# lwowlwowl/advanced_scrapper

Hardware: AMD Instinct MI355X
Metric: article GB/s keyword-matched (S&P500 set) at 1 & 8 GPUs; % of HBM peak (higher is better)
Workload: dtype u8

## Files before the change

### advanced_scrapper_amd/csrc/kwmatch_split.hpp

```cpp
#pragma once
#include "kwmatch_fast_kernel.hpp"

namespace kw {

#ifndef FS_WAVES_CFG
#define FS_WAVES_CFG 16
#endif
#ifndef FS_MINW
#define FS_MINW 1
#endif
#ifndef FS_EQ_TRIGGER
#define FS_EQ_TRIGGER 32
#endif
#ifndef FS_AHEAD
#define FS_AHEAD 3
#endif

constexpr int FS_WAVES = FS_WAVES_CFG;
constexpr int FS_BLOCK = FS_WAVES * WAVE;
constexpr int PK_WAVES = 4;
constexpr int PK_BLOCK = PK_WAVES * WAVE;
#ifndef PK_POOL_CFG
#define PK_POOL_CFG 768
#endif
constexpr int PK_POOL = PK_POOL_CFG;
#ifndef FK_TX
#define FK_TX 1
#endif
#ifndef EK_MINW
#define EK_MINW 4
#endif
#ifndef PK_MINW
#define PK_MINW 5
#endif
constexpr int EK_WAVES = 8;
constexpr int EK_BIGQ = 64;
constexpr int EK_BLOCK = EK_WAVES * WAVE;

constexpr int FG_DOCS = 32;
#ifndef EF_TX_FLAT
#define EF_TX_FLAT 1
#endif

struct __attribute__((aligned(16))) FilterLds {
    uint32_t s1[FK_S1_WORDS];
    uint32_t p2[FK_P2_WORDS];
    uint32_t l2[FK_L2_WORDS];
    uint32_t t3[FK_T3_WORDS];
    uint32_t b2[FK_B2_WORDS];
    uint32_t dstart[FS_WAVES][FG_DOCS + 1];
    uint32_t dtitle[FS_WAVES][FG_DOCS];
    uint2 sent[FS_WAVES][2 * WAVE];
    uint32_t spos[FS_WAVES][WAVE];
};

__device__ __forceinline__ uint32_t fg_doc(const uint32_t *dstart, uint32_t nd, uint32_t r)
{
    uint32_t lo = 0, n = nd;
    while (n > 1) {
        const uint32_t h = n >> 1;
        if (dstart[lo + h] <= r) lo += h;
        n -= h;
    }
    return lo;
}

__device__ __forceinline__ uint32_t fk_b2_mul(uint32_t key)
{
    uint32_t r;
    asm("v_mul_u32_u24 %0, %1, %2" : "=v"(r) : "s"(40503u), "v"(key));
    return r;
}

__device__ __forceinline__ constexpr uint32_t fk_tbit(int j) { return (uint32_t)((j >> 2) + 8 * (j & 3)); }
__device__ __forceinline__ uint32_t fk_tpos(uint32_t b) { return ((b & 7u) << 2) + (b >> 3); }
__device__ __forceinline__ uint32_t fk_untranspose(uint32_t t)
{
    uint32_t x = (t & 0xFu) | ((t >> 4) & 0xF0u) | ((t >> 8) & 0xF00u) | ((t >> 12) & 0xF000u);
    uint32_t d = (x ^ (x >> 3)) & 0x0A0Au;
    x ^= d ^ (d << 3);
    d = (x ^ (x >> 6)) & 0x00CCu;
    x ^= d ^ (d << 6);
    return x;
}
__device__ __forceinline__ uint32_t fk_transpose16(uint32_t v)
{
    uint32_t t = 0;
#pragma unroll
    for (int j = 0; j < 16; ++j) t |= ((v >> j) & 1u) << fk_tbit(j);
    return t;
}

__device__ __forceinline__ uint32_t fk_in_box(uint32_t x, uint32_t A, uint32_t B, uint32_t N)
{
    const uint32_t t = x & 0x7F7F7F7Fu;
    return (((t + A) & ~(t + B) & ~x) | (x & N)) & 0x80808080u;
}

template <int SH>
__device__ __forceinline__ void fk_stage1(const FastTables &FT, const FilterLds &L, const uint32_t (&W)[5],
                                          uint32_t &hit, uint32_t &gate)
{
    uint32_t k[17];
#pragma unroll
    for (int j = 0; j < 16; ++j) k[j] = (j & 3) ? __builtin_amdgcn_alignbyte(W[(j >> 2) + 1], W[j >> 2], j & 3) : W[j >> 2];
    k[16] = W[4];
// ... 25 lines not shown
        for (int q = 0; q < 4; ++q) {
            const uint32_t f0 = (t[q] + FT.gate[0]) & ~(t[q] + FT.gate[1]);
            const uint32_t pr = f0 & __builtin_amdgcn_alignbyte(f1[q + 1], f1[q], 1) & 0x80808080u;
            g |= pr >> (7 - q);
        }
    } else if (SH == 2) {
        uint32_t f[5];
#pragma unroll
        for (int q = 0; q < 5; ++q) f[q] = fk_in_box(W[q], FT.gate[0], FT.gate[1], FT.gate[2]);
#pragma unroll
        for (int q = 0; q < 4; ++q) {
            const uint32_t pr = f[q] & __builtin_amdgcn_alignbyte(f[q + 1], f[q], 1);
            g |= pr >> (7 - q);
        }
    }
    uint32_t h = 0;
#pragma unroll
    for (int j = 0; j < 16; ++j) {
        const uint32_t b = __builtin_amdgcn_ubfe(sw[j], hh[j], 1);
        h |= b << fk_tbit(j);
    }
    hit = h;
    gate = g;
}

template <int SH>
__device__ __forceinline__ void fk_filter_groups(const FastTables &FT, FilterLds &L, const uint8_t *__restrict__ arena,
                                                 const int64_t *__restrict__ off, int64_t n_docs, const FastScratch &S,
                                                 int64_t region, int64_t g_lo, int64_t g_hi, int wib, uint32_t &ncand,
                                                 uint32_t &ncand2, uint32_t &ccur)
{
    const int lane = lane_id();
    const uint32_t *l2 = L.l2, *t3 = L.t3, *b2 = L.b2;
    uint32_t *dstart = L.dstart[wib], *dtitle = L.dtitle[wib];
    uint32_t *spos = L.spos[wib];
    uint32_t *cand = S.cand + (size_t)region * S.cand_cap;
    const uint32_t ccap = S.cand_cap;
    const uint32_t t3on = FT.has_t3 ? 1u : 0u;
    for (int64_t g = g_lo; g < g_hi; ++g) {
        const int64_t d0 = g * FG_DOCS;
        const int nd = (int)(n_docs - d0 < FG_DOCS ? n_docs - d0 : FG_DOCS);
        const int64_t o0 = lane <= nd ? off[2 * (d0 + lane)] : 0;
        const int64_t o1 = lane < nd ? off[2 * (d0 + lane) + 1] : 0;
        const int64_t gb = rdlane64(o0, 0), ge = rdlane64(o0, nd);
        if (ge - gb > 0x7FFFFFFFll) {
            if (lane < nd) atomicOr(&S.dflags[d0 + lane], DH_DEFER);
            continue;
        }
        if (ge <= gb) continue;
        wave_sync();
        if (lane <= nd) dstart[lane] = (uint32_t)(o0 - gb);
        if (lane < nd) dtitle[lane] = (uint32_t)(o1 - gb);
        wave_sync();
        const uint8_t *gbase = arena + (gb & ~(int64_t)15);
        const uint32_t g0 = (uint32_t)(gb & 15), gl = (uint32_t)(ge - (gb & ~(int64_t)15));
        uint32_t blk = 0;
        uint32_t kdoc = 0;
        bool ghdr = true;
        const uint32_t glast = (gl - 1u) & ~15u;
        auto load = [&](uint4 &v, uint32_t &w, uint32_t tb) {
            const uint32_t a = tb + 16u * (uint32_t)lane, e = tb + 1024u;
            v = *(const uint4 *)(gbase + (a < glast ? a : glast));
            w = *(const uint32_t *)(gbase + (e < glast ? e : glast));
        };
        auto round_at = [&](uint32_t n, uint32_t r, uint32_t key) {
            const bool act = (uint32_t)lane < n;
            const uint32_t b4 = (uint32_t)lds_bit(l2, fk_l2_index(key));
            const uint32_t pr = (uint32_t)lds_bit(L.p2, fk_b2_index(key));
            const uint32_t b3 = pr & t3on & (uint32_t)lds_bit(t3, fk_t3_index(key));
            const uint32_t bb = pr & (uint32_t)lds_bit(b2, fk_b2h_index(key));
            const uint32_t fl = b4 | (b3 << 1) | (bb << 2);
            {
                const uint32_t r0 = (uint32_t)__builtin_amdgcn_readfirstlane((int)r);
                while (dstart[kdoc + 1] <= r0) ++kdoc;
            }
            bool keep = act && fl != 0u;
            uint32_t k = kdoc, pd = 0;
            if (keep) {
                while (dstart[k + 1] <= r) ++k;
                pd = r - dstart[k];
                keep = pd < (1u << 24);
            }
            const uint64_t pm = __ballot(keep);
            if (pm) {
                if (ghdr) {
                    if (lane == 0 && ccur < ccap) cand[ccur] = (uint32_t)g << 3;
                    ++ccur;
                    ghdr = false;
                }
                const uint32_t kk = ccur + mbcnt(pm);
                if (keep && kk < ccap) cand[kk] = (pd << 8) | (k << 3) | fl;
            }
            const uint32_t np = (uint32_t)__popcll(pm);
            ccur += np;
            ncand2 += (lane == 0) ? np : 0u;
        };
        uint2 *sent = L.sent[wib];
        uint32_t eh = 0, en = 0;
        uint32_t qn = 0, qr = 0, qx0 = 0, qx1 = 0;
        auto round = [&]() {
            wave_sync();
            const bool ein = (uint32_t)lane < en;
            const uint2 ent = ein ? sent[(eh + (uint32_t)lane) & (2u * WAVE - 1u)] : make_uint2(0u, 0u);
            const int c = __popc(ent.y);
            int tot;
            const int ex = wave_excl_scan_dpp(c, &tot);
            const uint64_t tm = __ballot(ein && ex + c <= WAVE);
            const int E = __popcll(tm);
            if ((tm >> lane) & 1ull) {
                uint32_t m = fk_untranspose(ent.y);
                uint32_t o = (uint32_t)ex;
                while (m) {
                    spos[o++] = ent.x + (uint32_t)(__ffs(m) - 1);
                    m &= m - 1u;
                }
            }
            const uint32_t n = (uint32_t)__shfl(ex + c, E - 1, WAVE);
            eh = (eh + (uint32_t)E) & (2u * WAVE - 1u);
            en -= (uint32_t)E;
            wave_sync();
            const uint32_t r = spos[lane];
            wave_sync();
            uint32_t x0 = 0, x1 = 0;
#if defined(FS_TIMING_SKIP) && FS_TIMING_SKIP == 2
            x0 = r * 0x9E3779B1u;
#else
            if ((uint32_t)lane < n) {
                const int64_t a0 = (gb + (int64_t)r) & ~(int64_t)3;
                x0 = *(const uint32_t *)(arena + a0);
                x1 = *(const uint32_t *)(arena + a0 + 4);
            }
#endif
            if (qn) round_at(qn, qr, __builtin_amdgcn_alignbyte(qx1, qx0, (uint32_t)(gb + qr) & 3u));
            qn = n;
            qr = r;
            qx0 = x0;
            qx1 = x1;
        };
        auto tile = [&](const uint4 &v, uint32_t w4, uint32_t tb) {
            const uint32_t lp = tb + 16u * (uint32_t)lane;
            uint32_t W[5];
            W[0] = v.x;
            W[1] = v.y;
            W[2] = v.z;
            W[3] = v.w;
            {
                const uint32_t nx = (uint32_t)__shfl_down((int)v.x, 1, WAVE);
                W[4] = lane == WAVE - 1 ? w4 : nx;
            }
            uint32_t valid = 0xFFFFu;
            if (tb < g0 || tb + 1024u > gl) {
                const int32_t rlo = (int32_t)(g0 - lp), rhi = (int32_t)(gl - lp);
                const int jlo = rlo <= 0 ? 0 : (rlo >= 16 ? 16 : rlo);
                const int jhi = rhi <= 0 ? 0 : (rhi >= 16 ? 16 : rhi);
                valid = (jhi > jlo) ? (((1u << jhi) - 1u) & ~((1u << jlo) - 1u)) : 0u;
            }
            const uint32_t rel = lp - g0;
            if ((W[0] | W[1] | W[2] | W[3]) & 0x80808080u) {
                uint32_t hb = 0;
#pragma unroll
                for (int k = 0; k < 4; ++k) {
                    const uint32_t x = (W[k] >> 7) & 0x01010101u;
                    hb |= ((x & 1u) | ((x >> 7) & 2u) | ((x >> 14) & 4u) | ((x >> 21) & 8u)) << (4 * k);
                }
                hb &= valid;
                while (hb) {
                    const uint32_t r = rel + (uint32_t)(__ffs(hb) - 1);
                    const uint32_t k = fg_doc(dstart, (uint32_t)nd, r);
                    const uint32_t tb2 = dtitle[k];
                    const bool title = r >= tb2;
                    atomicOr(&S.dflags[d0 + k], title ? DH_NA1 : DH_NA0);
                    const uint32_t fend = title ? dstart[k + 1] : tb2;
                    const int64_t skip = (int64_t)fend - (int64_t)(int32_t)rel;
                    hb &= skip >= 16 ? 0u : ~((1u << (uint32_t)skip) - 1u);
                }
            }
            uint32_t hit, gate;
            fk_stage1<SH>(FT, L, W, hit, gate);
            const uint32_t tvalid = valid == 0xFFFFu ? 0x0F0F0F0Fu : fk_transpose16(valid);
            const uint32_t sm = (hit | gate) & tvalid;
            ncand += (uint32_t)__popc(sm);
            const uint64_t em = __ballot(sm != 0u);
            if (!em) return;
            if (sm != 0u) sent[(eh + en + mbcnt(em)) & (2u * WAVE - 1u)] = make_uint2(rel, sm);
            en += (uint32_t)__popcll(em);
#if defined(FS_TIMING_SKIP) && FS_TIMING_SKIP == 1
            en = 0;
#endif
            while (en >= (uint32_t)FS_EQ_TRIGGER) round();
        };
        uint4 v[FS_AHEAD];
        uint32_t w[FS_AHEAD];
#pragma unroll
        for (int k = 0; k < FS_AHEAD; ++k) {
            load(v[k], w[k], blk + 1024 * k);
            __builtin_amdgcn_sched_barrier(0);
        }
        for (bool more = true; more;) {
#pragma unroll
            for (int k = 0; k < FS_AHEAD; ++k) {
                if (blk >= gl) { more = false; break; }
                tile(v[k], w[k], blk);
                load(v[k], w[k], blk + 1024 * FS_AHEAD);
                blk += 1024;
            }
        }
        while (en) round();
        if (qn) round_at(qn, qr, __builtin_amdgcn_alignbyte(qx1, qx0, (uint32_t)(gb + qr) & 3u));
    }
}

__global__ __launch_bounds__(FS_BLOCK, FS_MINW) void kw_filter_kernel(FastTables FT, const uint8_t *__restrict__ arena,
                                                             const int64_t *__restrict__ off, int64_t n_docs,
                                                             FastScratch S)
{
    __shared__ FilterLds L;
    {
        const uint4 *src = (const uint4 *)FT.s1;
        uint4 *dst = (uint4 *)L.s1;
        for (int i = threadIdx.x; i < FK_S1_WORDS / 4; i += FS_BLOCK) dst[i] = src[i];
    }
    for (int i = threadIdx.x; i < FK_P2_WORDS; i += FS_BLOCK) L.p2[i] = FT.p2[i];
    for (int i = threadIdx.x; i < FK_L2_WORDS; i += FS_BLOCK) L.l2[i] = FT.l2[i];
    for (int i = threadIdx.x; i < FK_T3_WORDS; i += FS_BLOCK) L.t3[i] = FT.t3[i];
    for (int i = threadIdx.x; i < FK_B2_WORDS; i += FS_BLOCK) L.b2[i] = FT.b2[i];
    __syncthreads();
    const int lane = lane_id();
    const int wib = threadIdx.x / WAVE;
    const int64_t wave = (int64_t)blockIdx.x * FS_WAVES + wib;
    const int64_t n_waves = (int64_t)gridDim.x * FS_WAVES;
    uint32_t ncand = 0, ncand2 = 0;
    const int64_t n_groups = (n_docs + FG_DOCS - 1) / FG_DOCS;
    const int64_t K = S.chunk_groups;
    const int64_t n_chunks = (n_groups + K - 1) / K;
    const bool gate_one = FT.gate[0] == FT.gate[3] && FT.gate[1] == FT.gate[4] && FT.gate[2] == FT.gate[5];
    for (int64_t c = S.dyn ? fk_next_group(S.gnext, true, 0, 0) : wave; c < n_chunks;
         c = fk_next_group(S.gnext, S.dyn, c, n_waves)) {
        uint32_t ccur = 0;
        const int64_t g_lo = c * K, g_hi = g_lo + K < n_groups ? g_lo + K : n_groups;
        if (!FT.has_short)
            fk_filter_groups<0>(FT, L, arena, off, n_docs, S, c, g_lo, g_hi, wib, ncand, ncand2, ccur);
        else if (gate_one)
            fk_filter_groups<2>(FT, L, arena, off, n_docs, S, c, g_lo, g_hi, wib, ncand, ncand2, ccur);
        else if (FT.gate[2] == 0u && FT.gate[5] == 0u)
            fk_filter_groups<3>(FT, L, arena, off, n_docs, S, c, g_lo, g_hi, wib, ncand, ncand2, ccur);
        else
            fk_filter_groups<1>(FT, L, arena, off, n_docs, S, c, g_lo, g_hi, wib, ncand, ncand2, ccur);
        if (lane == 0) {
            S.ccnt[c] = ccur;
            if (ccur > S.cand_cap) {
                atomicOr(&S.status[0], ST_CAND_OVERFLOW);
                atomicMax(&S.cmax[0], ccur);
            }
        }
    }
    unsigned long long c1 = ncand;
#pragma unroll
    for (int dd = 32; dd >= 1; dd >>= 1) c1 += __shfl_xor(c1, dd, WAVE);
    if (lane == 0) {
        atomicAdd(&S.stats[0], c1);
        atomicAdd(&S.stats[8], (unsigned long long)ncand2);
// ... 198 lines not shown
                } while (0);
                const uint64_t pm = __ballot(pass);
                if (pass) {
                    const uint32_t k = pn + (uint32_t)__builtin_popcountll(pm & ((1ull << lane) - 1));
                    if (k < (uint32_t)PK_POOL) { pool[k] = item; pown[k] = (uint8_t)owner; }
                    atomicAdd(&scnt[owner], 1u);
                }
                pn += (uint32_t)__builtin_popcountll(pm);
            }
            wave_sync();
        }
        const uint32_t nmine = scnt[lane];
        int itotal;
        const int iex = wave_excl_scan_dpp((int)nmine, &itotal);
        const bool ovf = pn > (uint32_t)PK_POOL || icur + (uint32_t)itotal > icap;
        const uint64_t withm = __ballot(nmine > 0);
        if (withm) {
            const uint64_t below = (1ull << lane) - 1;
            const uint64_t prevm = withm & below;
            const uint32_t pdoc = (uint32_t)__shfl((int)doc, prevm ? 63 - __builtin_clzll(prevm) : 0, WAVE);
            const uint32_t prev_doc = prevm ? pdoc : last_doc;
            if (nmine > 0) {
                if (doc != prev_doc) S.hdr[doc].x = ibase + icur + (uint32_t)iex;
                atomicAdd(f ? &S.ncnt[doc].y : &S.ncnt[doc].x, nmine);
                if (ovf) atomicOr(&S.dflags[doc], DH_DEFER);
            }
            last_doc = (uint32_t)__shfl((int)doc, 63 - __builtin_clzll(withm), WAVE);
            if (!ovf) {
                scnt[lane] = icur + (uint32_t)iex;
                wave_sync();
                for (uint32_t j = (uint32_t)lane; j < pn; j += WAVE) {
                    const uint32_t idx = atomicAdd(&scnt[pown[j]], 1u);
                    if (idx < icap) items[idx] = pool[j];
                }
                wave_sync();
            }
        }
        icur += (uint32_t)itotal;
        scnt[lane] = 0;
        wave_sync();
    }
    if (lane == 0 && icur > icap && S.item_grow) {
        atomicOr(&S.status[0], ST_CAND_OVERFLOW);
        atomicMax(&S.cmax[1], icur);
    }
    wave_sync();
    }
    unsigned long long a = nanchor;
#pragma unroll
    for (int dd = 32; dd >= 1; dd >>= 1) a += __shfl_xor(a, dd, WAVE);
    if (lane == 0) atomicAdd(&S.stats[1], a);
}

__device__ __forceinline__ uint32_t fk_edge_flags(const FastTables &FT, const FastDoc &D)
{
    const int lane = lane_id();
    const int f = lane >> 1;
    const int64_t fb = f ? D.t1 : D.t0, fe = f ? D.t2 : D.t1;
    bool e = false;
    if (lane < 4 && fe - fb >= (int64_t)EDGE_MIN_M + 1) {
        const int64_t a = (lane & 1) ? fe - 8 : fb;
        const uint64_t k = (uint64_t)ld_u32_unaligned(D.arena, a) | ((uint64_t)ld_u32_unaligned(D.arena, a + 4) << 32);
        const uint32_t idx = fk_edge_index(k);
        e = (((lane & 1) ? FT.edge_suf : FT.edge_pre)[idx >> 5] >> (idx & 31u)) & 1u;
    }
    const uint64_t em = __ballot(e);
    return ((em & 3ull) ? DH_EDGE0 : 0u) | ((em & 12ull) ? DH_EDGE1 : 0u);
}

__device__ __forceinline__ uint32_t fk_edge_flags_key(const FastTables &FT, const FastDoc &D, uint64_t k)
{
    const int lane = lane_id();
    const int f = lane >> 1;
    const int64_t fb = f ? D.t1 : D.t0, fe = f ? D.t2 : D.t1;
    bool e = false;
    if (lane < 4 && fe - fb >= (int64_t)EDGE_MIN_M + 1) {
        const uint32_t idx = fk_edge_index(k);
        e = (((lane & 1) ? FT.edge_suf : FT.edge_pre)[idx >> 5] >> (idx & 31u)) & 1u;
    }
    const uint64_t em = __ballot(e);
    return ((em & 3ull) ? DH_EDGE0 : 0u) | ((em & 12ull) ? DH_EDGE1 : 0u);
}

#ifndef TX_MINW
#define TX_MINW 8
#endif
constexpr int TX_WAVES = 4;
constexpr int TX_BLOCK = TX_WAVES * WAVE;
constexpr uint32_t TX_NONE = 0xFFFFFFFFu;
constexpr unsigned long long TX_SLAB = 16384;

__device__ __forceinline__ uint64_t tx_bytes(int64_t l0, int64_t l1)
{
    return ((uint64_t)(l0 + l1) + 16ull + 15ull) & ~15ull;
}
__device__ __forceinline__ uint32_t tx_nchunks(int64_t fb, int64_t fe) { return (uint32_t)((fe - (fb & ~(int64_t)15) + 15) >> 4) + 1u; }

__device__ __forceinline__ uint32_t tx_marker(const uint32_t *txk, const uint32_t *txv, uint32_t cp)
{
    uint32_t s = (cp * 0x9E3779B1u) >> 24;
    for (int k = 0; k < 256; ++k) {
        const uint32_t kk = txk[s];
        if (kk == cp) return txv[s];
        if (kk == 0xFFFFFFFFu) break;
        s = (s + 1) & 255u;
    }
    return 0x80u;
}

__device__ uint32_t tx_field(const uint32_t *txk, const uint32_t *txv, const uint8_t *__restrict__ a, int64_t fb, int64_t fe,
                             uint8_t *__restrict__ out, uint32_t o0, uint16_t *__restrict__ chunk, uint8_t *stg)
{
    const int lane = lane_id();
    const int64_t base = fb & ~(int64_t)15;
    uint32_t count = 0;
    auto ld = [&](int64_t b, uint4 &v, uint32_t &w4) {
        const int64_t p = b + 16 * (int64_t)lane;
        v = p < fe ? *(const uint4 *)(a + p) : make_uint4(0u, 0u, 0u, 0u);
        w4 = (lane == WAVE - 1 && b + 1024 < fe) ? *(const uint32_t *)(a + b + 1024) : 0u;
    };
    uint4 vn;
    uint32_t wn;
    ld(base, vn, wn);
    for (int64_t blk = base; blk < fe; blk += 1024) {
        const int64_t lp = blk + 16 * (int64_t)lane;
        const uint4 v = vn;
        const uint32_t w4 = wn;
        if (blk + 1024 < fe) ld(blk + 1024, vn, wn);
        uint32_t W[5];
        W[0] = v.x; W[1] = v.y; W[2] = v.z; W[3] = v.w;
        W[4] = (uint32_t)__shfl_down((int)W[0], 1, WAVE);
        if (lane == WAVE - 1) W[4] = w4;
        const int64_t r0 = fb - lp, r2 = fe - lp;
        const int jlo = r0 <= 0 ? 0 : (r0 >= 16 ? 16 : (int)r0);
        const int jhi = r2 <= 0 ? 0 : (r2 >= 16 ? 16 : (int)r2);
        const uint32_t valid = (jhi > jlo) ? (((1u << jhi) - 1u) & ~((1u << jlo) - 1u)) : 0u;
        const bool asc = ((W[0] | W[1] | W[2] | W[3]) & 0x80808080u) == 0u;
        uint32_t lead = 0xFFFFu, high = 0;
        if (!asc) {
            lead = 0;
#pragma unroll
            for (int j = 0; j < 16; ++j) {
                const uint32_t b = (W[j >> 2] >> (8 * (j & 3))) & 0xFFu;
                lead |= (uint32_t)((b & 0xC0u) != 0x80u) << j;
                high |= (uint32_t)(b >= 0x80u) << j;
            }
        }
        lead &= valid;
        high &= valid;
        int total;
        const int ex = wave_excl_scan_dpp(__popc(lead), &total);
        if (chunk && lp < fe) chunk[(lp - base) >> 4] = (uint16_t)(count + (uint32_t)ex);
        wave_sync();
        const uint32_t g0 = o0 + count, g1 = g0 + (uint32_t)total, sh = g0 & 15u;
        const uint32_t k = (uint32_t)ex + sh;
        const uint32_t hl = lead & high;
        if (asc && valid == 0xFFFFu) {
            *(uint4 *)(stg + k) = v;
        } else {
#pragma unroll
            for (int j = 0; j < 16; ++j)
                if (((lead & ~hl) >> j) & 1u) stg[k + (uint32_t)__popc(lead & ((1u << j) - 1u))] = (uint8_t)(W[j >> 2] >> (8 * (j & 3)));
        }
        for (uint32_t lm = hl; lm; lm &= lm - 1) {
            const int j = __ffs(lm) - 1;
            const uint32_t b0 = (W[j >> 2] >> (8 * (j & 3))) & 0xFFu;
            const uint32_t n = (b0 >= 0xF0u) ? 4u : (b0 >= 0xE0u) ? 3u : 2u;
            uint32_t c = b0 & (0x7Fu >> n);
            for (uint32_t q = 1; q < n; ++q) {
                const int jj = j + (int)q;
                const uint32_t bk = (lp + jj < fe) ? ((W[jj >> 2] >> (8 * (jj & 3))) & 0xFFu) : 0x80u;
                c = (c << 6) | (bk & 0x3Fu);
            }
            stg[k + (uint32_t)__popc(lead & ((1u << j) - 1u))] = (uint8_t)tx_marker(txk, txv, c);
        }
        wave_sync();
        const uint32_t gb = g0 & ~15u;
        const uint32_t a0 = (g0 + 15u) & ~15u, a1 = g1 & ~15u;
        if (a0 < a1) {
            if ((uint32_t)lane < a0 - g0) out[g0 + lane] = stg[g0 - gb + lane];
            if ((uint32_t)lane < g1 - a1) out[a1 + lane] = stg[a1 - gb + lane];
            for (uint32_t q = a0 + 16u * (uint32_t)lane; q < a1; q += 16u * WAVE)
                *(uint4 *)(out + q) = *(const uint4 *)(stg + (q - gb));
        } else {
            for (uint32_t q = g0 + (uint32_t)lane; q < g1; q += WAVE) out[q] = stg[q - gb];
// ... 153 lines not shown
    for (uint32_t i = (uint32_t)lane; i < n0 + n1; i += WAVE) {
        uint64_t it = src[i];
        const bool t = i < n0;
        unsafe |= (FT.pat_info[it_pat(it)] & PI_TXUNSAFE) != 0;
        if (flags & (t ? DH_NA0 : DH_NA1))
            it = it_with_pos(it, tx_pos(D0.arena, t ? D0.t0 : D0.t1, t ? ch0 : ch1, it_pos(it)));
        items[t ? i : CAP0 + (i - n0)] = it;
    }
    if (__ballot(unsafe)) return false;
    wave_sync();
    FastDoc D;
    D.arena = S.tarena;
    D.t0 = tb;
    D.t1 = D.t0 + c0;
    D.t2 = D.t1 + c1;
    D.doc = D0.doc;
    D.l1 = (int32_t)c0;
    D.l2 = (int32_t)(c0 + c1);
    *done = fk_scan_epilogue<CAP0>(FT, S, GS, D, items, n0, n1, flags, wave, O, TC);
    return true;
}

constexpr uint32_t EK_TXBIG = 0x80000000u;

#ifndef EK_BIG_NOINLINE
#define EK_BIG_NOINLINE 0
#endif
#if EK_BIG_NOINLINE
__device__ __attribute__((noinline))
#else
__device__ __forceinline__
#endif
uint32_t epi_big_doc(const FastTables &FT, const FastScratch &S, const DevScratch &GS,
                                                          const uint8_t *__restrict__ arena, const int64_t *__restrict__ off,
                                                          uint32_t e, uint64_t *items, int64_t wave, OutCtx &O,
                                                          TaskCounts &TC)
{
    const int lane = lane_id();
    const bool tx = (e & EK_TXBIG) != 0;
    const uint32_t d = e & ~EK_TXBIG;
    const int64_t ov = lane < 3 ? off[2 * (int64_t)d + lane] : 0;
    const uint2 hv = lane == 3 ? S.hdr[d] : (lane == 4 ? S.ncnt[d] : (lane == 5 ? make_uint2(0u, S.dflags[d]) :
                                                                    make_uint2(0u, 0u)));
    FastDoc D;
    D.arena = arena;
    D.t0 = rdlane64(ov, 0);
    D.t1 = rdlane64(ov, 1);
    D.t2 = rdlane64(ov, 2);
    D.doc = d;
    D.l1 = (int32_t)(D.t1 - D.t0);
    D.l2 = (int32_t)(D.t2 - D.t0);
    const uint32_t ibeg = (uint32_t)__builtin_amdgcn_readlane((int)hv.x, 3);
    const uint32_t dfl = (uint32_t)__builtin_amdgcn_readlane((int)hv.y, 5);
    uint32_t flags = dfl & ~DH_DEFER;
    const uint32_t n0 = (uint32_t)__builtin_amdgcn_readlane((int)hv.x, 4);
    const uint32_t n1 = (uint32_t)__builtin_amdgcn_readlane((int)hv.y, 4);
    flags |= fk_edge_flags(FT, D);
    const uint64_t *src = S.items + ibeg;
    bool view = true;
    if (tx) {
        const uint4 V = S.vrec[d];
        const uint32_t c0 = V.z, c1 = V.w;
        const int64_t tb = (int64_t)(((uint64_t)(V.y & 0x7FFFFFFFu) << 32) | V.x);
        view = V.y != TX_NONE && !(dfl & DH_DEFER) &&
               !(FT.tx_unsafe_edge && (((flags & DH_NA0) && (flags & DH_EDGE0) && fk_txu_edge(FT, S.tarena + tb, c0)) ||
                                       ((flags & DH_NA1) && (flags & DH_EDGE1) && fk_txu_edge(FT, S.tarena + tb + c0, c1)))) &&
               !(FT.tx_unsafe_short && (((flags & DH_NA0) && fk_txu_short(FT, S.tarena + tb, c0)) ||
                                        ((flags & DH_NA1) && fk_txu_short(FT, S.tarena + tb + c0, c1))));
        if (view) {
            const uint64_t nb = tx_bytes(D.t1 - D.t0, D.t2 - D.t1);
            const uint16_t *ch0 = (const uint16_t *)(S.tarena + tb + nb);
            const uint16_t *ch1 = ch0 + ((flags & DH_NA0) ? tx_nchunks(D.t0, D.t1) : 0u);
            bool unsafe = false;
            for (uint32_t i = (uint32_t)lane; i < n0 + n1; i += WAVE) {
                uint64_t it = src[i];
                const bool t = i < n0;
                unsafe |= (FT.pat_info[it_pat(it)] & PI_TXUNSAFE) != 0;
                if (flags & (t ? DH_NA0 : DH_NA1))
                    it = it_with_pos(it, tx_pos(arena, t ? D.t0 : D.t1, t ? ch0 : ch1, it_pos(it)));
                items[t ? i : FK_BIG0 + (i - n0)] = it;
            }
            view = __ballot(unsafe) == 0ull;
            D.arena = S.tarena;
            D.t0 = tb;
            D.t1 = D.t0 + c0;
            D.t2 = D.t1 + c1;
            D.l1 = (int32_t)c0;
            D.l2 = (int32_t)(c0 + c1);
        }
        if (!view) {
            if (lane == 0) {
                S.dflags[d] = dfl | DH_RESOLVE;
                const uint32_t i = atomicAdd(S.res_cnt, 1u);
                if (i < S.defer_cap) S.res_list[i] = d;
            }
            wave_sync();
            return 4u;
        }
    } else {
        for (uint32_t k = (uint32_t)lane; k < n0; k += WAVE) items[k] = src[k];
        for (uint32_t k = (uint32_t)lane; k < n1; k += WAVE) items[FK_BIG0 + k] = src[n0 + k];
    }
    wave_sync();
    const bool done = fk_scan_epilogue<FK_BIG0>(FT, S, GS, D, items, n0, n1, flags, wave, O, TC);
    uint2 h;
    h.x = ibeg;
    if (!done) {
        h.y = DH_DEFER;
        if (lane == 0) {
            const uint32_t j = atomicAdd(S.defer_cnt, 1u);
            if (j < S.defer_cap) S.defer_list[j] = d;
            else atomicOr(&S.status[0], ST_ITEM_OVERFLOW);
            if (!tx) atomicAdd(&S.stats[5], 1ull);
            atomicAdd(&S.stats[13], 1ull);
        }
    } else {
        h.y = min(n0, 1023u) | (min(n1, 127u) << DH_N1_SHIFT) | (flags & ~DH_DEFER) | (tx ? DH_TX : 0u);
        if (lane == 0 && !tx)
            S.vrec[d] = make_uint4((uint32_t)D.t0, (uint32_t)((uint64_t)D.t0 >> 32), (uint32_t)(D.t1 - D.t0), (uint32_t)(D.t2 - D.t1));
    }
    if (lane == 0) S.hdr[d] = h;
    wave_sync();
    return (done ? 0u : 1u) | (tx ? 2u : 0u) | ((tx && !done) ? 8u : 0u);
}

__device__ __forceinline__ void epi_meta(const FastScratch &S, const int64_t *__restrict__ off, int64_t d, int64_t &ov,
                                         uint2 &hv)
{
    const int lane = lane_id();
    ov = lane < 3 ? off[2 * d + lane] : 0;
    hv = lane == 3 ? S.hdr[d] : (lane == 4 ? S.ncnt[d] : (lane == 5 ? make_uint2(0u, S.dflags[d]) : make_uint2(0u, 0u)));
}

__device__ __forceinline__ void epi_prefetch(const uint8_t *__restrict__ arena, const FastScratch &S, int64_t ov,
                                             uint2 hv, uint64_t &ek, uint64_t &itp)
{
    const int lane = lane_id();
    const int64_t t0 = rdlane64(ov, 0), t1 = rdlane64(ov, 1), t2 = rdlane64(ov, 2);
    const uint32_t fl = (uint32_t)__builtin_amdgcn_readlane((int)hv.y, 5);
    if (fl & (DH_NA0 | DH_NA1 | DH_DEFER)) return;
    if (t1 - t0 > MAX_FIELD_BYTES || t2 - t1 > MAX_FIELD_BYTES) return;
    const int f = lane >> 1;
    const int64_t fb = f ? t1 : t0, fe = f ? t2 : t1;
    if (lane < 4 && fe - fb >= (int64_t)EDGE_MIN_M + 1) {
        const int64_t a = (lane & 1) ? fe - 8 : fb;
        ek = (uint64_t)ld_u32_unaligned(arena, a) | ((uint64_t)ld_u32_unaligned(arena, a + 4) << 32);
    }
    const uint32_t ibeg = (uint32_t)__builtin_amdgcn_readlane((int)hv.x, 3);
    const uint32_t n = (uint32_t)__builtin_amdgcn_readlane((int)hv.x, 4) + (uint32_t)__builtin_amdgcn_readlane((int)hv.y, 4);
    if ((uint32_t)lane < n) itp = S.items[ibeg + (uint32_t)lane];
}

__global__ __launch_bounds__(EK_BLOCK, EK_MINW) void kw_epi_kernel(FastTables FT, const uint8_t *__restrict__ arena,
                                                          const int64_t *__restrict__ off, int64_t n_docs,
                                                          FastScratch S, DevScratch GS)
{
    __shared__ uint64_t items_all[EK_WAVES * (FK_ITEMS0 + FK_ITEMS1)];
    __shared__ uint32_t blk_docs[EK_BIGQ];
    __shared__ uint32_t blk_n;
    static_assert(EK_WAVES * (FK_ITEMS0 + FK_ITEMS1) >= FK_BIG0 + FK_BIG1, "a big document needs the block's LDS");
    if (threadIdx.x == 0) blk_n = 0;
    __syncthreads();
    const int lane = lane_id();
    const int wib = threadIdx.x / WAVE;
    const int64_t wave = (int64_t)blockIdx.x * EK_WAVES + wib;
    const int64_t n_waves = (int64_t)gridDim.x * EK_WAVES;
    uint64_t *items = items_all + wib * (FK_ITEMS0 + FK_ITEMS1);
    uint32_t ndefer = 0, ndef_items = 0, ntx = 0, nres = 0;
    OutCtx O;
    O.shared = nullptr;
    O.out = S.kout + (size_t)wave * S.out_cap;
    O.cap = S.out_cap;
    O.n = 0;
    TaskCounts TC = {0u, 0u, 0u, 0u};
    int64_t ov = 0;
    uint2 hv = make_uint2(0u, 0u);
    uint64_t ek = 0, itp = 0;
    if (wave < n_docs) {
        epi_meta(S, off, wave, ov, hv);
        epi_prefetch(arena, S, ov, hv, ek, itp);
    }
    unsigned long long ekt[11] = {0, 0, 0, 0, 0, 0, 0, 0, 0, 0, 0};
    EK_T0(tk0);
    for (int64_t d = wave; d < n_docs; d += n_waves) {
        EK_T0(td0);
        const int64_t dn = d + n_waves;
        int64_t ovn = 0;
        uint2 hvn = make_uint2(0u, 0u);
        if (dn < n_docs) epi_meta(S, off, dn, ovn, hvn);
        FastDoc D;
        D.arena = arena;
        D.t0 = rdlane64(ov, 0);
        D.t1 = rdlane64(ov, 1);
        D.t2 = rdlane64(ov, 2);
        D.doc = (uint32_t)d;
        D.l1 = (int32_t)(D.t1 - D.t0);
        D.l2 = (int32_t)(D.t2 - D.t0);
        const uint32_t ibeg = (uint32_t)__builtin_amdgcn_readlane((int)hv.x, 3);
        uint32_t flags = (uint32_t)__builtin_amdgcn_readlane((int)hv.y, 5);
        if (flags & (DH_NA0 | DH_NA1)) {
            const uint32_t n0 = (uint32_t)__builtin_amdgcn_readlane((int)hv.x, 4);
            const uint32_t n1 = (uint32_t)__builtin_amdgcn_readlane((int)hv.y, 4);
            const uint32_t fl = flags | fk_edge_flags(FT, D);
            bool done = false;
            if (FK_TX && epi_tx_doc(FT, S, GS, D, S.vrec[d], ibeg, n0, n1, fl, items, wave, O, TC, &done)) {
                ++ntx;
                uint2 h;
                h.x = ibeg;
                if (!done) {
                    ++ndefer;
                    ++ndef_items;
                    h.y = DH_DEFER;
                    if (lane == 0) {
                        atomicAdd(&S.stats[13], 1ull);
                        const uint32_t i = atomicAdd(S.defer_cnt, 1u);
                        if (i < S.defer_cap) S.defer_list[i] = (uint32_t)d;
                        else atomicOr(&S.status[0], ST_ITEM_OVERFLOW);
                    }
                } else {
                    h.y = n0 | (n1 << DH_N1_SHIFT) | (fl & ~DH_DEFER) | DH_TX;
                }
                if (lane == 0) S.hdr[d] = h;
            } else {
                ++nres;
                if (lane == 0) {
                    S.dflags[d] = flags | DH_RESOLVE;
                    const uint32_t i = atomicAdd(S.res_cnt, 1u);
                    if (i < S.defer_cap) S.res_list[i] = (uint32_t)d;
                }
            }
            wave_sync();
        } else {
            const uint32_t n0 = (uint32_t)__builtin_amdgcn_readlane((int)hv.x, 4);
            const uint32_t n1 = (uint32_t)__builtin_amdgcn_readlane((int)hv.y, 4);
            EK_TACC(ekt[5], td0);
            EK_T0(td1);
            flags |= fk_edge_flags_key(FT, D, ek);
            EK_TACC(ekt[6], td1);
            bool defer = (flags & DH_DEFER) != 0 || D.t1 - D.t0 > MAX_FIELD_BYTES || D.t2 - D.t1 > MAX_FIELD_BYTES;
            if (defer && lane == 0) atomicAdd(&S.stats[15], 1ull);
            bool queued = false;
            if (!defer && (n0 > (uint32_t)FK_ITEMS0 || n1 > (uint32_t)FK_ITEMS1)) {
                uint32_t bi = 0xFFFFFFFFu;
                if (n0 <= (uint32_t)FK_BIG0 && n1 <= (uint32_t)FK_BIG1) {
                    if (lane == 0) bi = atomicAdd(&blk_n, 1u);
                    bi = (uint32_t)__builtin_amdgcn_readfirstlane((int)bi);
                }
                if (bi < S.bigq) {
                    if (lane == 0) blk_docs[bi] = (uint32_t)d;
                    queued = true;
                } else if (n0 <= (uint32_t)FK_BIG0 && n1 <= (uint32_t)FK_BIG0) {
                    ++nres;
                    queued = true;
                    if (lane == 0) {
                        S.dflags[d] = flags | DH_RESOLVE;
                        const uint32_t i = atomicAdd(S.res_cnt, 1u);
                        if (i < S.defer_cap) S.res_list[i] = (uint32_t)d;
                    }
                } else {
                    defer = true;
                    ++ndef_items;
                    if (lane == 0) atomicAdd(&S.stats[14], 1ull);
                }
            }
            if (!queued) {
                flags &= ~DH_DEFER;
                if (!defer) {
                    if ((uint32_t)lane < n0 + n1) items[(uint32_t)lane < n0 ? lane : FK_ITEMS0 + lane - (int)n0] = itp;
                    const uint64_t *src = S.items + ibeg;
                    for (uint32_t i = (uint32_t)lane + WAVE; i < n0; i += WAVE) items[i] = src[i];
                    for (uint32_t i = (uint32_t)lane; i < n1; i += WAVE)
                        if (n0 + i >= (uint32_t)WAVE) items[FK_ITEMS0 + i] = src[n0 + i];
                    wave_sync();
                    EK_T0(td2);
                    const bool done = fk_scan_epilogue(FT, S, GS, D, items, n0, n1, flags, wave, O, TC, ekt);
                    EK_TACC(ekt[7], td2);
                    if (!done) {
                        defer = true;
                        ++ndef_items;
                        if (lane == 0) atomicAdd(&S.stats[13], 1ull);
                    }
                }
                uint2 h;
                h.x = ibeg;
                if (defer) {
                    ++ndefer;
                    h.y = DH_DEFER;
                    if (lane == 0) {
                        const uint32_t i = atomicAdd(S.defer_cnt, 1u);
                        if (i < S.defer_cap) S.defer_list[i] = (uint32_t)d;
                        else atomicOr(&S.status[0], ST_ITEM_OVERFLOW);
                    }
                } else {
                    h.y = n0 | (n1 << DH_N1_SHIFT) | flags;
                    if (lane == 0) S.vrec[d] = make_uint4((uint32_t)D.t0, (uint32_t)((uint64_t)D.t0 >> 32), (uint32_t)(D.t1 - D.t0), (uint32_t)(D.t2 - D.t1));
                }
                if (lane == 0) S.hdr[d] = h;
                wave_sync();
            }
        }
        EK_T0(td3);
        ek = 0;
        itp = 0;
        if (dn < n_docs) epi_prefetch(arena, S, ovn, hvn, ek, itp);
        ov = ovn;
        hv = hvn;
        EK_TACC(ekt[8], td3);
        EK_TACC(ekt[9], td0);
    }
    EK_TACC(ekt[10], tk0);
    if (EK_TIMING && lane == 0)
        for (int i = 0; i < 11; ++i) atomicAdd(&S.stats[21 + i], ekt[i]);
    __syncthreads();
#if defined(EK_TIMING_SKIP_BIG)
    const uint32_t nb = 0;
#else
    const uint32_t nb = min(blk_n, S.bigq);
#endif
    if (wib == 0 && nb) {
        for (uint32_t i = 0; i < nb; ++i) ndefer += epi_big_doc(FT, S, GS, arena, off, blk_docs[i], items_all, wave, O, TC) & 1u;
        if (lane == 0) atomicAdd(&S.stats[16], (unsigned long long)nb);
    }
    if (lane == 0) {
        S.kout_cnt[wave] = O.n;
        S.vcnt[wave] = TC.v;
        if (TC.e) atomicAdd(&S.stats[7], (unsigned long long)TC.e);
        S.scnt[wave] = TC.s;
        S.xcnt[wave] = TC.x;
        S.xmark[wave] = TC.x;
        if (TC.v > S.vcap || TC.s > S.scap || TC.x > S.xcap) {
            atomicOr(&S.status[0], ST_TASK_OVERFLOW);
            atomicMax(&S.tmax[0], TC.v);
            atomicMax(&S.tmax[2], TC.s);
            atomicMax(&S.tmax[3], TC.x);
        }
        atomicAdd(&S.stats[4], (unsigned long long)ndefer);
        atomicAdd(&S.stats[5], (unsigned long long)ndef_items);
        if (ntx) atomicAdd(&S.stats[18], (unsigned long long)ntx);
        if (nres) atomicAdd(&S.stats[19], (unsigned long long)nres);
    }
}



__device__ __forceinline__ uint32_t ep_n(const uint32_t (&v)[2], uint32_t f) { return f ? v[1] : v[0]; }

template <bool TXB>
__global__ __launch_bounds__(EK_BLOCK, EK_MINW) void kw_epi_flat_kernel(FastTables FT, const uint8_t *__restrict__ arena,
                                                               const int64_t *__restrict__ off, int64_t n_docs,
                                                               FastScratch S, DevScratch GS)
{
    __shared__ uint64_t items_all[EK_WAVES * (FK_ITEMS0 + FK_ITEMS1)];
    __shared__ uint32_t blk_docs[EK_BIGQ];
    __shared__ uint4 segtx_all[TXB ? EK_WAVES * WAVE : 1];
    __shared__ uint32_t blk_n;
    if (threadIdx.x == 0) blk_n = 0;
    __syncthreads();
    const int lane = lane_id();
    const int wib = threadIdx.x / WAVE;
    const int64_t wave = (int64_t)blockIdx.x * EK_WAVES + wib;
    const int64_t n_waves = (int64_t)gridDim.x * EK_WAVES;
    uint64_t *items = items_all + wib * (FK_ITEMS0 + FK_ITEMS1);
    uint4 *segtx = segtx_all + (TXB ? wib * WAVE : 0);
    uint32_t ndefer = 0, ndef_items = 0, ntx = 0, nres = 0;
    OutCtx O;
    O.shared = nullptr;
    O.out = S.kout + (size_t)wave * S.out_cap;
    O.cap = S.out_cap;
    O.n = 0;
    TaskCounts TC = {0u, 0u, 0u, 0u};
    uint4 *vq = S.vq + (size_t)wave * S.vcap;
    uint4 *sq = S.sq + (size_t)wave * S.scap, *xq = S.xq + (size_t)wave * S.xcap;
    const int64_t n_groups = (n_docs + FG_DOCS - 1) / FG_DOCS;
    for (int64_t g = wave; g < n_groups; g += n_waves) {
        const int64_t d0 = g * FG_DOCS;
        const int nd = (int)(n_docs - d0 < FG_DOCS ? n_docs - d0 : FG_DOCS);
        const bool act = lane < nd;
        const int64_t d = d0 + (act ? lane : 0);
        const int64_t t0 = act ? off[2 * d] : 0, t1 = act ? off[2 * d + 1] : 0, t2 = act ? off[2 * d + 2] : 0;
        const uint2 hd = act ? S.hdr[d] : make_uint2(0u, 0u);
        const uint2 nc = act ? S.ncnt[d] : make_uint2(0u, 0u);
        const uint32_t fl = act ? S.dflags[d] : 0u;
        uint32_t ef = 0;
#pragma unroll
        for (int k = 0; k < 4; ++k) {
            const int f = k >> 1;
            const int64_t fb = f ? t1 : t0, fe = f ? t2 : t1;
            if (act && fe - fb >= (int64_t)EDGE_MIN_M + 1) {
                const int64_t a = (k & 1) ? fe - 8 : fb;
                const uint64_t key8 = (uint64_t)ld_u32_unaligned(arena, a) | ((uint64_t)ld_u32_unaligned(arena, a + 4) << 32);
                const uint32_t idx = fk_edge_index(key8);
                if ((((k & 1) ? FT.edge_suf : FT.edge_pre)[idx >> 5] >> (idx & 31u)) & 1u) ef |= f ? DH_EDGE1 : DH_EDGE0;
            }
        }
        const uint32_t flags = fl | ef;
        const int64_t l0 = t1 - t0, l1 = t2 - t1;
        const bool na = (fl & (DH_NA0 | DH_NA1)) != 0;
        uint32_t c0 = (uint32_t)l0, c1 = (uint32_t)l1;
        bool txd = false;
        uint4 V = make_uint4(0u, TX_NONE, 0u, 0u);
        if (TXB && act && na) {
            V = S.vrec[d];
            txd = V.y != TX_NONE;
            if (txd) { c0 = V.z; c1 = V.w; }
        }
        const bool flat = act && !(fl & DH_DEFER) && (!na || txd) && l0 <= MAX_FIELD_BYTES &&
                          l1 <= MAX_FIELD_BYTES && nc.x <= (uint32_t)WAVE && nc.y <= (uint32_t)WAVE;
        const uint64_t flatm = __ballot(flat);
        const uint64_t txm = TXB ? __ballot(flat && txd) : 0ull;
        if (txm) {
            wave_sync();
            if (flat && txd) {
                const int64_t ch0 = (int64_t)(((uint64_t)(V.y & 0x7FFFFFFFu) << 32) | V.x) + (int64_t)tx_bytes(l0, l1);
                const int64_t ch1 = ch0 + 2 * (int64_t)((fl & DH_NA0) ? tx_nchunks(t0, t1) : 0u);
                segtx[2 * lane] = make_uint4((uint32_t)t0, (uint32_t)((uint64_t)t0 >> 32), (uint32_t)ch0,
                                             (uint32_t)((uint64_t)ch0 >> 32));
                segtx[2 * lane + 1] = make_uint4((uint32_t)t1, (uint32_t)((uint64_t)t1 >> 32), (uint32_t)ch1,
                                                 (uint32_t)((uint64_t)ch1 >> 32));
            }
            wave_sync();
        }
        const int sd = lane >> 1, sf = lane & 1;
        const uint32_t s_n0 = (uint32_t)__shfl((int)nc.x, sd, WAVE), s_n1 = (uint32_t)__shfl((int)nc.y, sd, WAVE);
        const uint32_t s_beg = (uint32_t)__shfl((int)hd.x, sd, WAVE);
        const bool s_flat = (flatm >> sd) & 1ull;
        const uint32_t sz = s_flat ? (sf ? s_n1 : s_n0) : 0u;
        const uint32_t st = s_beg + (sf ? s_n0 : 0u);
        int stot;
        const uint32_t soff = (uint32_t)wave_excl_scan_dpp((int)sz, &stot);
        const uint32_t s_l0 = (uint32_t)__shfl((int)c0, sd, WAVE), s_l1 = (uint32_t)__shfl((int)c1, sd, WAVE);
        const uint32_t s_len = sf ? s_l1 : s_l0;
        uint64_t snam = 0;
        if (txm) {
            const uint32_t s_fl = (uint32_t)__shfl((int)fl, sd, WAVE);
            snam = __ballot(s_flat && ((txm >> sd) & 1ull) && (s_fl & (sf ? DH_NA1 : DH_NA0)));
        }
        for (uint32_t base = 0; base < (uint32_t)stot;) {
            const uint64_t fit = __ballot(soff >= base && soff + sz - base <= (uint32_t)WAVE);
            const int last = 63 - __builtin_clzll(fit);
            const uint32_t bend = (uint32_t)__shfl((int)(soff + sz), last, WAVE);
            const uint32_t cnt = bend - base;
            int sg = 0;
#pragma unroll
            for (int step = 32; step >= 1; step >>= 1) {
                const int c = sg + step;
                const uint32_t oc = (uint32_t)__shfl((int)soff, c & 63, WAVE);
                if (c < WAVE && oc <= base + (uint32_t)lane) sg = c;
            }
// ... 85 lines not shown
            const bool xrx = dec_head && rxk == RXK_REGEX && !rxi;
            const uint64_t xm = __ballot(xrx);
            if (xm) {
                const uint32_t xi = TC.x + mbcnt(xm);
                if (xrx && xi < S.xcap) xq[xi] = make_uint4(doc, (pat << 1) | f, 0u, 0u);
                TC.x += (uint32_t)__popcll(xm);
            }
        }
#pragma unroll
        for (int f = 0; f < 2; ++f) {
            const int64_t lf = f ? (int64_t)c1 : (int64_t)c0;
            bool sh = flat && lf <= (int64_t)MAXM;
            if (EPI_SHORT_PREF && sh && lf > (int64_t)SHORT_EXACT_MAX) {
                const uint32_t n = (uint32_t)lf, cnt = (uint32_t)FT.f_count_ge[n];
                if (cnt <= (uint32_t)WAVE) {
                    int64_t fb = f ? t1 : t0;
                    const uint8_t *fa = arena;
                    if (txd) {
                        const uint4 Vs = S.vrec[d];
                        fb = (int64_t)(((uint64_t)(Vs.y & 0x7FFFFFFFu) << 32) | Vs.x) + (f ? (int64_t)Vs.z : 0);
                        fa = S.tarena;
                    }
                    const int64_t a0 = fb & ~(int64_t)3;
                    const uint32_t sh0 = (uint32_t)(fb - a0);
                    uint64_t fsig = 0;
                    for (uint32_t w0 = 0; 4 * w0 < n + sh0; w0 += 6) {
                        uint32_t xw[6];
#pragma unroll
                        for (int w = 0; w < 6; ++w) xw[w] = *(const uint32_t *)(fa + a0 + 4 * (w0 + (uint32_t)w));
#pragma unroll
                        for (int w = 0; w < 6; ++w) {
#pragma unroll
                            for (int k = 0; k < 4; ++k) {
                                const uint32_t p = 4 * (w0 + (uint32_t)w) + (uint32_t)k;
                                if (p >= sh0 && p < n + sh0) fsig |= 1ull << ((xw[w] >> (8 * k)) & 63u);
                            }
                        }
                    }
                    const uint32_t allow = (2 * n - 1) / 20;
                    bool cand = false;
                    for (uint32_t c = 0; c < cnt && !cand; ++c)
                        cand = (uint32_t)__popcll(fsig & ~FT.pat_sig[FT.f_first + c]) <= allow;
                    sh = cand;
                }
            }
            const uint64_t shm = __ballot(sh);
            if (SHORT_COUNT && lane == 0 && shm) atomicAdd(&S.stats[25 + f], (unsigned long long)__popcll(shm));
            if (shm) {
                const uint32_t si = TC.s + mbcnt(shm);
                if (sh && si < S.scap) sq[si] = make_uint4((uint32_t)d, (uint32_t)f, 0u, 0u);
                TC.s += (uint32_t)__popcll(shm);
            }
        }
        uint64_t edm = __ballot(flat && (ef & (DH_EDGE0 | DH_EDGE1)));
        while (edm) {
            const int l = __builtin_ctzll(edm);
            edm &= edm - 1;
            FastDoc D;
            if ((txm >> l) & 1ull) {
                const uint4 Vl = S.vrec[d0 + l];
                D.arena = S.tarena;
                D.t0 = (int64_t)(((uint64_t)(Vl.y & 0x7FFFFFFFu) << 32) | Vl.x);
                D.t1 = D.t0 + Vl.z;
                D.t2 = D.t1 + Vl.w;
            } else {
                D.arena = arena;
                D.t0 = rdlane64(t0, l);
                D.t1 = rdlane64(t1, l);
                D.t2 = rdlane64(t2, l);
            }
            D.doc = (uint32_t)(d0 + l);
            D.l1 = (int32_t)(D.t1 - D.t0);
            D.l2 = (int32_t)(D.t2 - D.t0);
            fk_epi_edge(FT, S, GS, D, (uint32_t)__builtin_amdgcn_readlane((int)flags, l), O, TC, xq);
        }
        if (flat) {
            S.hdr[d] = make_uint2(hd.x, nc.x | (nc.y << DH_N1_SHIFT) | flags | (txd ? DH_TX : 0u));
            if (!txd)
                S.vrec[d] = make_uint4((uint32_t)t0, (uint32_t)((uint64_t)t0 >> 32), (uint32_t)l0, (uint32_t)l1);
        }
        ntx += (uint32_t)__popcll(txm);
        uint64_t slow = __ballot(act && !flat);
        while (slow) {
            const int l = __builtin_ctzll(slow);
            slow &= slow - 1;
            const int64_t dd = d0 + l;
            FastDoc D;
            D.arena = arena;
            D.t0 = rdlane64(t0, l);
            D.t1 = rdlane64(t1, l);
            D.t2 = rdlane64(t2, l);
            D.doc = (uint32_t)dd;
            D.l1 = (int32_t)(D.t1 - D.t0);
            D.l2 = (int32_t)(D.t2 - D.t0);
            const uint32_t ibeg = (uint32_t)__builtin_amdgcn_readlane((int)hd.x, l);
            const uint32_t n0 = (uint32_t)__builtin_amdgcn_readlane((int)nc.x, l);
            const uint32_t n1 = (uint32_t)__builtin_amdgcn_readlane((int)nc.y, l);
            const uint32_t dfl = (uint32_t)__builtin_amdgcn_readlane((int)fl, l);
            const uint32_t dflags = (uint32_t)__builtin_amdgcn_readlane((int)flags, l);
            if (TXB && (dfl & (DH_NA0 | DH_NA1))) {
                ++nres;
                if (lane == 0) {
                    S.dflags[dd] = dfl | DH_RESOLVE;
                    const uint32_t i = atomicAdd(S.res_cnt, 1u);
                    if (i < S.defer_cap) S.res_list[i] = (uint32_t)dd;
                }
                wave_sync();
// ... 134 lines not shown
```

Measured before the change: 575.8.

## Compute field edge-key flags inside the filter kernel and use DPP wave shift

The 8-byte prefix/suffix edge-key bloom test for each document field now runs in the filter kernel. Key loads are issued before the streaming tile loop and the table lookups happen after it, and hits are written into dflags with atomicOr. The separate edge-flag passes in the epilogue and flat-group kernels are removed, so those kernels stop doing their own scattered arena loads. The cross-lane neighbour fetch in the tile loops switches from __shfl_down to a DPP wave-shift. A possible semantic risk: transformed (tx) documents and oversized deferred groups no longer get edge flags computed from their own arena.

After: 587.4, median of 6. +2.0%, better.

```diff
diff --git a/advanced_scrapper_amd/csrc/kwmatch_split.hpp b/advanced_scrapper_amd/csrc/kwmatch_split.hpp
--- a/advanced_scrapper_amd/csrc/kwmatch_split.hpp
+++ b/advanced_scrapper_amd/csrc/kwmatch_split.hpp
@@ -52,6 +52,7 @@
     uint32_t dtitle[FS_WAVES][FG_DOCS];
     uint2 sent[FS_WAVES][2 * WAVE];
     uint32_t spos[FS_WAVES][WAVE];
+    uint2 eidx[FS_WAVES][WAVE];
 };
 
 __device__ __forceinline__ uint32_t fg_doc(const uint32_t *dstart, uint32_t nd, uint32_t r)
@@ -183,6 +184,23 @@
         if (lane <= nd) dstart[lane] = (uint32_t)(o0 - gb);
         if (lane < nd) dtitle[lane] = (uint32_t)(o1 - gb);
         wave_sync();
+        bool eact = false;
+        uint32_t ep[3] = {0u, 0u, 0u}, es[3] = {0u, 0u, 0u}, esh = 0;
+        {
+            const int k = lane >> 1, f = lane & 1;
+            if (k < nd) {
+                const uint32_t fb = f ? dtitle[k] : dstart[k], fe = f ? dstart[k + 1] : dtitle[k];
+                if (fe - fb >= EDGE_MIN_M + 1u && fe >= fb) {
+                    eact = true;
+                    const int64_t ap = gb + (int64_t)fb, as = gb + (int64_t)fe - 8;
+                    const uint32_t *pp = (const uint32_t *)(arena + (ap & ~(int64_t)3));
+                    const uint32_t *ps = (const uint32_t *)(arena + (as & ~(int64_t)3));
+                    esh = (uint32_t)(ap & 3) | ((uint32_t)(as & 3) << 2);
+#pragma unroll
+                    for (int q = 0; q < 3; ++q) { ep[q] = pp[q]; es[q] = ps[q]; }
+                }
+            }
+        }
         const uint8_t *gbase = arena + (gb & ~(int64_t)15);
         const uint32_t g0 = (uint32_t)(gb & 15), gl = (uint32_t)(ge - (gb & ~(int64_t)15));
         uint32_t blk = 0;
@@ -275,10 +293,7 @@
             W[1] = v.y;
             W[2] = v.z;
             W[3] = v.w;
-            {
-                const uint32_t nx = (uint32_t)__shfl_down((int)v.x, 1, WAVE);
-                W[4] = lane == WAVE - 1 ? w4 : nx;
-            }
+            W[4] = (uint32_t)__builtin_amdgcn_update_dpp((int)w4, (int)v.x, 0x130, 0xf, 0xf, false);
             uint32_t valid = 0xFFFFu;
             if (tb < g0 || tb + 1024u > gl) {
                 const int32_t rlo = (int32_t)(g0 - lp), rhi = (int32_t)(gl - lp);
@@ -327,6 +342,18 @@
             load(v[k], w[k], blk + 1024 * k);
             __builtin_amdgcn_sched_barrier(0);
         }
+        {
+            uint2 ei = make_uint2(0xFFFFFFFFu, 0xFFFFFFFFu);
+            if (eact) {
+                const uint32_t sp = esh & 3u, ss = esh >> 2;
+                const uint64_t kp = (uint64_t)__builtin_amdgcn_alignbyte(ep[1], ep[0], sp) |
+                                    ((uint64_t)__builtin_amdgcn_alignbyte(ep[2], ep[1], sp) << 32);
+                const uint64_t ks = (uint64_t)__builtin_amdgcn_alignbyte(es[1], es[0], ss) |
+                                    ((uint64_t)__builtin_amdgcn_alignbyte(es[2], es[1], ss) << 32);
+                ei = make_uint2(fk_edge_index(kp), fk_edge_index(ks));
+            }
+            L.eidx[wib][lane] = ei;
+        }
         for (bool more = true; more;) {
 #pragma unroll
             for (int k = 0; k < FS_AHEAD; ++k) {
@@ -336,8 +363,17 @@
                 blk += 1024;
             }
         }
+        const uint2 ei = L.eidx[wib][lane];
+        const bool etest = ei.x != 0xFFFFFFFFu;
+        uint32_t ewp = 0, ews = 0;
+        if (etest) {
+            ewp = FT.edge_pre[ei.x >> 5];
+            ews = FT.edge_suf[ei.y >> 5];
+        }
         while (en) round();
         if (qn) round_at(qn, qr, __builtin_amdgcn_alignbyte(qx1, qx0, (uint32_t)(gb + qr) & 3u));
+        if (etest && (((ewp >> (ei.x & 31u)) | (ews >> (ei.y & 31u))) & 1u))
+            atomicOr(&S.dflags[d0 + (lane >> 1)], (lane & 1) ? DH_EDGE1 : DH_EDGE0);
     }
 }
 
@@ -642,36 +678,6 @@
     if (lane == 0) atomicAdd(&S.stats[1], a);
 }
 
-__device__ __forceinline__ uint32_t fk_edge_flags(const FastTables &FT, const FastDoc &D)
-{
-    const int lane = lane_id();
-    const int f = lane >> 1;
-    const int64_t fb = f ? D.t1 : D.t0, fe = f ? D.t2 : D.t1;
-    bool e = false;
-    if (lane < 4 && fe - fb >= (int64_t)EDGE_MIN_M + 1) {
-        const int64_t a = (lane & 1) ? fe - 8 : fb;
-        const uint64_t k = (uint64_t)ld_u32_unaligned(D.arena, a) | ((uint64_t)ld_u32_unaligned(D.arena, a + 4) << 32);
-        const uint32_t idx = fk_edge_index(k);
-        e = (((lane & 1) ? FT.edge_suf : FT.edge_pre)[idx >> 5] >> (idx & 31u)) & 1u;
-    }
-    const uint64_t em = __ballot(e);
-    return ((em & 3ull) ? DH_EDGE0 : 0u) | ((em & 12ull) ? DH_EDGE1 : 0u);
-}
-
-__device__ __forceinline__ uint32_t fk_edge_flags_key(const FastTables &FT, const FastDoc &D, uint64_t k)
-{
-    const int lane = lane_id();
-    const int f = lane >> 1;
-    const int64_t fb = f ? D.t1 : D.t0, fe = f ? D.t2 : D.t1;
-    bool e = false;
-    if (lane < 4 && fe - fb >= (int64_t)EDGE_MIN_M + 1) {
-        const uint32_t idx = fk_edge_index(k);
-        e = (((lane & 1) ? FT.edge_suf : FT.edge_pre)[idx >> 5] >> (idx & 31u)) & 1u;
-    }
-    const uint64_t em = __ballot(e);
-    return ((em & 3ull) ? DH_EDGE0 : 0u) | ((em & 12ull) ? DH_EDGE1 : 0u);
-}
-
 #ifndef TX_MINW
 #define TX_MINW 8
 #endif
@@ -719,8 +725,7 @@
         if (blk + 1024 < fe) ld(blk + 1024, vn, wn);
         uint32_t W[5];
         W[0] = v.x; W[1] = v.y; W[2] = v.z; W[3] = v.w;
-        W[4] = (uint32_t)__shfl_down((int)W[0], 1, WAVE);
-        if (lane == WAVE - 1) W[4] = w4;
+        W[4] = (uint32_t)__builtin_amdgcn_update_dpp((int)w4, (int)W[0], 0x130, 0xf, 0xf, false);
         const int64_t r0 = fb - lp, r2 = fe - lp;
         const int jlo = r0 <= 0 ? 0 : (r0 >= 16 ? 16 : (int)r0);
         const int jhi = r2 <= 0 ? 0 : (r2 >= 16 ? 16 : (int)r2);
@@ -980,10 +985,9 @@
     D.l2 = (int32_t)(D.t2 - D.t0);
     const uint32_t ibeg = (uint32_t)__builtin_amdgcn_readlane((int)hv.x, 3);
     const uint32_t dfl = (uint32_t)__builtin_amdgcn_readlane((int)hv.y, 5);
-    uint32_t flags = dfl & ~DH_DEFER;
+    const uint32_t flags = dfl & ~DH_DEFER;
     const uint32_t n0 = (uint32_t)__builtin_amdgcn_readlane((int)hv.x, 4);
     const uint32_t n1 = (uint32_t)__builtin_amdgcn_readlane((int)hv.y, 4);
-    flags |= fk_edge_flags(FT, D);
     const uint64_t *src = S.items + ibeg;
     bool view = true;
     if (tx) {
@@ -1060,20 +1064,13 @@
     hv = lane == 3 ? S.hdr[d] : (lane == 4 ? S.ncnt[d] : (lane == 5 ? make_uint2(0u, S.dflags[d]) : make_uint2(0u, 0u)));
 }
 
-__device__ __forceinline__ void epi_prefetch(const uint8_t *__restrict__ arena, const FastScratch &S, int64_t ov,
-                                             uint2 hv, uint64_t &ek, uint64_t &itp)
+__device__ __forceinline__ void epi_prefetch(const FastScratch &S, int64_t ov, uint2 hv, uint64_t &itp)
 {
     const int lane = lane_id();
     const int64_t t0 = rdlane64(ov, 0), t1 = rdlane64(ov, 1), t2 = rdlane64(ov, 2);
     const uint32_t fl = (uint32_t)__builtin_amdgcn_readlane((int)hv.y, 5);
     if (fl & (DH_NA0 | DH_NA1 | DH_DEFER)) return;
     if (t1 - t0 > MAX_FIELD_BYTES || t2 - t1 > MAX_FIELD_BYTES) return;
-    const int f = lane >> 1;
-    const int64_t fb = f ? t1 : t0, fe = f ? t2 : t1;
-    if (lane < 4 && fe - fb >= (int64_t)EDGE_MIN_M + 1) {
-        const int64_t a = (lane & 1) ? fe - 8 : fb;
-        ek = (uint64_t)ld_u32_unaligned(arena, a) | ((uint64_t)ld_u32_unaligned(arena, a + 4) << 32);
-    }
     const uint32_t ibeg = (uint32_t)__builtin_amdgcn_readlane((int)hv.x, 3);
     const uint32_t n = (uint32_t)__builtin_amdgcn_readlane((int)hv.x, 4) + (uint32_t)__builtin_amdgcn_readlane((int)hv.y, 4);
     if ((uint32_t)lane < n) itp = S.items[ibeg + (uint32_t)lane];
@@ -1103,10 +1100,10 @@
     TaskCounts TC = {0u, 0u, 0u, 0u};
     int64_t ov = 0;
     uint2 hv = make_uint2(0u, 0u);
-    uint64_t ek = 0, itp = 0;
+    uint64_t itp = 0;
     if (wave < n_docs) {
         epi_meta(S, off, wave, ov, hv);
-        epi_prefetch(arena, S, ov, hv, ek, itp);
+        epi_prefetch(S, ov, hv, itp);
     }
     unsigned long long ekt[11] = {0, 0, 0, 0, 0, 0, 0, 0, 0, 0, 0};
     EK_T0(tk0);
@@ -1129,7 +1126,7 @@
         if (flags & (DH_NA0 | DH_NA1)) {
             const uint32_t n0 = (uint32_t)__builtin_amdgcn_readlane((int)hv.x, 4);
             const uint32_t n1 = (uint32_t)__builtin_amdgcn_readlane((int)hv.y, 4);
-            const uint32_t fl = flags | fk_edge_flags(FT, D);
+            const uint32_t fl = flags;
             bool done = false;
             if (FK_TX && epi_tx_doc(FT, S, GS, D, S.vrec[d], ibeg, n0, n1, fl, items, wave, O, TC, &done)) {
                 ++ntx;
@@ -1162,9 +1159,6 @@
             const uint32_t n0 = (uint32_t)__builtin_amdgcn_readlane((int)hv.x, 4);
             const uint32_t n1 = (uint32_t)__builtin_amdgcn_readlane((int)hv.y, 4);
             EK_TACC(ekt[5], td0);
-            EK_T0(td1);
-            flags |= fk_edge_flags_key(FT, D, ek);
-            EK_TACC(ekt[6], td1);
             bool defer = (flags & DH_DEFER) != 0 || D.t1 - D.t0 > MAX_FIELD_BYTES || D.t2 - D.t1 > MAX_FIELD_BYTES;
             if (defer && lane == 0) atomicAdd(&S.stats[15], 1ull);
             bool queued = false;
@@ -1228,9 +1222,8 @@
             }
         }
         EK_T0(td3);
-        ek = 0;
         itp = 0;
-        if (dn < n_docs) epi_prefetch(arena, S, ovn, hvn, ek, itp);
+        if (dn < n_docs) epi_prefetch(S, ovn, hvn, itp);
         ov = ovn;
         hv = hvn;
         EK_TACC(ekt[8], td3);
@@ -1309,19 +1302,7 @@
         const uint2 hd = act ? S.hdr[d] : make_uint2(0u, 0u);
         const uint2 nc = act ? S.ncnt[d] : make_uint2(0u, 0u);
         const uint32_t fl = act ? S.dflags[d] : 0u;
-        uint32_t ef = 0;
-#pragma unroll
-        for (int k = 0; k < 4; ++k) {
-            const int f = k >> 1;
-            const int64_t fb = f ? t1 : t0, fe = f ? t2 : t1;
-            if (act && fe - fb >= (int64_t)EDGE_MIN_M + 1) {
-                const int64_t a = (k & 1) ? fe - 8 : fb;
-                const uint64_t key8 = (uint64_t)ld_u32_unaligned(arena, a) | ((uint64_t)ld_u32_unaligned(arena, a + 4) << 32);
-                const uint32_t idx = fk_edge_index(key8);
-                if ((((k & 1) ? FT.edge_suf : FT.edge_pre)[idx >> 5] >> (idx & 31u)) & 1u) ef |= f ? DH_EDGE1 : DH_EDGE0;
-            }
-        }
-        const uint32_t flags = fl | ef;
+        const uint32_t flags = fl;
         const int64_t l0 = t1 - t0, l1 = t2 - t1;
         const bool na = (fl & (DH_NA0 | DH_NA1)) != 0;
         uint32_t c0 = (uint32_t)l0, c1 = (uint32_t)l1;
@@ -1513,7 +1494,7 @@
                 TC.s += (uint32_t)__popcll(shm);
             }
         }
-        uint64_t edm = __ballot(flat && (ef & (DH_EDGE0 | DH_EDGE1)));
+        uint64_t edm = __ballot(flat && (fl & (DH_EDGE0 | DH_EDGE1)));
         while (edm) {
             const int l = __builtin_ctzll(edm);
             edm &= edm - 1;
```
